# sjpark0905/DNA-LDPC-codes

Hardware: NVIDIA B200
Metric: decoded Gbit/s, n=18432 prprp (higher is better)
Workload: dtype f64

## Files before the change

dna-ldpc-codes_b200/csrc/bp_kernels.cuh:

```cuda
#pragma once
#include <cuda_runtime.h>
#include <stdint.h>

#include "bp_math.cuh"
#include "rng.cuh"

namespace dnaldpc {

constexpr int kFG = 32;

template <typename T> __device__ __forceinline__ T ld_stream(const T *p) { return __ldcs(p); }
template <typename T> __device__ __forceinline__ void st_stream(T *p, T v) { __stcs(p, v); }


template <typename T>
__device__ __noinline__ void row_slow_path(T *base, const T *lr_lane, const int32_t *cols, int deg, bool fresh) {
    auto pr_at = [&](int k) -> T { return fresh ? lr_lane[(size_t)cols[k] * kFG] : base[(size_t)k * kFG]; };
    T B = T(1);
    for (int k = deg - 1; k >= 0; k--) {
        T F = T(1);
        for (int m = 0; m < k; m++) F = mul_rn(F, check_factor_slow(pr_at(m)));
        const T dk = check_factor_slow(pr_at(k));
        base[(size_t)k * kFG] = check_to_bit_slow(mul_rn(F, B));
        B = mul_rn(B, dk);
// ... 324 lines not shown
    ck = __hiloint2double((int)w[17], (int)w[16]);
}

__device__ __forceinline__ int nth_set_bit8(uint32_t m, int r) {
    int f = 0;
#pragma unroll
    for (int q = 0; q < 8; q++) {
        if (q == r && m) f = __ffs(m) - 1;
        m &= m - 1;
    }
    return f;
}

constexpr int kTmWarps = 12;

template <int DC, int UR>
__global__ void __launch_bounds__(kTmWarps * 32, 1)
row_pass_tmem_kernel(double *__restrict__ msg, const double *__restrict__ lratio, const uint32_t *__restrict__ actw,
                     const uint32_t *__restrict__ freshw, const int32_t *__restrict__ col_idx, int M, int N, int E,
                     int g0, int G, unsigned int *__restrict__ job_counter, int l2_hint) {
    static_assert(DC % 8 == 0 && (DC / 8) * kTmBlockCols * (kTmWarps / 4) <= 512, "tensor-memory columns");
    constexpr uint32_t kTileBytes = DC * kFG * sizeof(double);
    constexpr int NB = DC / 8, NT = DC / 4, NI = (DC + 31) / 32;
    extern __shared__ __align__(128) unsigned char smem_raw[];
    const int lane = threadIdx.x & 31, warp = threadIdx.x >> 5;
    double *tile = reinterpret_cast<double *>(smem_raw) + (size_t)warp * DC * kFG;
    unsigned char *aux = smem_raw + (size_t)kTmWarps * DC * kFG * sizeof(double);
    uint64_t *bar = reinterpret_cast<uint64_t *>(aux) + warp;
    int *sidx = reinterpret_cast<int *>(aux + kTmWarps * sizeof(uint64_t)) + warp * DC;
    uint32_t *tm_slot = reinterpret_cast<uint32_t *>(aux + kTmWarps * sizeof(uint64_t) + (size_t)kTmWarps * DC * sizeof(int));
    const double *col = tile + lane;
    const uint64_t policy = l2_evict_first_policy();
    if (warp == 0) tmem_alloc_512(tm_slot);
    if (lane == 0) {
        mbar_init(bar, 1);
        mbar_fence_init();
    }
    asm volatile("tcgen05.fence::before_thread_sync;" ::: "memory");
    __syncthreads();
    asm volatile("tcgen05.fence::after_thread_sync;" ::: "memory");
    const uint32_t tm_base = *tm_slot;
    const uint32_t taddr = tm_base + ((uint32_t)((warp & 3) * 32) << 16) + (uint32_t)((warp >> 2) * NB * kTmBlockCols);
    const unsigned njobs = (unsigned)M * (unsigned)G;
    const int kq = lane >> 3, rk = lane & 7;
    uint32_t phase = 0;

    auto start_item = [&](int g, int e0, uint32_t act, uint32_t fw, double (&v)[NT]) {
        const uint32_t fresh_mask = fw & act;
        if ((act & ~fresh_mask) != 0 && lane == 0) {
            asm volatile("fence.proxy.async.shared::cta;" ::: "memory");
            mbar_expect_tx(bar, kTileBytes);
            if (l2_hint) tma_load_1d_hint(tile, msg + ((size_t)g * E + e0) * kFG, kTileBytes, bar, policy);
            else tma_load_1d(tile, msg + ((size_t)g * E + e0) * kFG, kTileBytes, bar);
        }
        if (fresh_mask != 0) {
            const bool mine = rk < __popc(fresh_mask);
            const int f = nth_set_bit8(fresh_mask, rk);
            const double *lr_base = lratio + (size_t)g * N * kFG;
#pragma unroll
            for (int t = 0; t < NT; t++) v[t] = mine ? lr_base[(size_t)sidx[t * 4 + kq] * kFG + f] : 0.0;
        }
    };
    auto claim_raw = [&]() -> unsigned {
        unsigned j = 0;
        if (lane == 0) j = atomicAdd(job_counter, 1u);
        return j;
    };

    unsigned job = __shfl_sync(0xffffffffu, claim_raw(), 0);
    unsigned job_n = __shfl_sync(0xffffffffu, claim_raw(), 0);
    int g = 0, e0 = 0;
    uint32_t act = 0, fw = 0;
    double v[NT];
    if (job < njobs) {
        g = g0 + (int)(job / (unsigned)M);
        e0 = (int)(job % (unsigned)M) * DC;
        for (int k = lane; k < DC; k += 32) sidx[k] = __ldg(col_idx + e0 + k);
        __syncwarp();
        act = actw[g]; fw = freshw[g];
        if (act != 0) start_item(g, e0, act, fw, v);
    }
    while (job < njobs) {
        const unsigned raw_nn = claim_raw();
        const bool valid_n = job_n < njobs;
        const int g_n = g0 + (int)(job_n / (unsigned)M), e0_n = (int)(job_n % (unsigned)M) * DC;
        uint32_t act_n = 0, fw_n = 0;
        int idx_n[NI];
#pragma unroll
        for (int q = 0; q < NI; q++) idx_n[q] = 0;
        if (valid_n) {
            act_n = actw[g_n]; fw_n = freshw[g_n];
#pragma unroll
            for (int q = 0; q < NI; q++)
                if (lane + 32 * q < DC) idx_n[q] = __ldg(col_idx + e0_n + lane + 32 * q);
        }
        const bool on = (act >> lane) & 1u, fresh = (fw >> lane) & 1u;
        double *base = msg + ((size_t)g * E + e0) * kFG + lane;
        const double *lr_lane = lratio + (size_t)g * N * kFG + lane;
        const int32_t *cols_cur = col_idx + e0;
        bool bad = false;
        if (act != 0) {
            const uint32_t fresh_mask = fw & act;
            if ((act & ~fresh_mask) != 0) {
                mbar_wait(bar, phase);
                phase ^= 1u;
            }
            if (fresh_mask != 0) {
                const int nf = __popc(fresh_mask);
                {
                    const bool mine = rk < nf;
                    const int f = nth_set_bit8(fresh_mask, rk);
#pragma unroll
                    for (int t = 0; t < NT; t++)
                        if (mine) tile[(t * 4 + kq) * kFG + f] = v[t];
                }
                for (int r0 = 8; r0 < nf; r0 += 8) {
                    const int r = r0 + rk;
                    const bool mine = r < nf;
                    const int f = mine ? (int)__fns(fresh_mask, 0, r + 1) : 0;
                    double w[NT];
#pragma unroll
                    for (int t = 0; t < NT; t++) w[t] = mine ? lr_lane[(size_t)sidx[t * 4 + kq] * kFG + (f - lane)] : 0.0;
#pragma unroll
                    for (int t = 0; t < NT; t++)
                        if (mine) tile[(t * 4 + kq) * kFG + f] = w[t];
                }
                __syncwarp();
            }
            double B = 1.0;
#pragma unroll(UR)
            for (int b = NB - 1; b >= 0; b--) {
                double d8[8];
                const double ckb = B;
#pragma unroll
                for (int kk = 7; kk >= 0; kk--) {
                    const double dk = check_factor(col[(b * 8 + kk) * kFG], bad);
                    d8[kk] = dk;
                    B = mul_rn(B, dk);
                }
                tmem_st_block(taddr + (uint32_t)(b * kTmBlockCols), d8, ckb);
            }
            asm volatile("tcgen05.wait::st.sync.aligned;" ::: "memory");
        }
        __syncwarp();
#pragma unroll
        for (int q = 0; q < NI; q++)
            if (lane + 32 * q < DC) sidx[lane + 32 * q] = idx_n[q];
        __syncwarp();
        if (valid_n && act_n != 0) start_item(g_n, e0_n, act_n, fw_n, v);
        if (on && bad) row_slow_path<double>(base, lr_lane, cols_cur, DC, fresh);
        if (act != 0) {
            double F = 1.0;
            const bool store = on && !bad;
#pragma unroll(UR)
            for (int b = 0; b < NB; b++) {
                double d8[8], Bv[8];
                tmem_ld_block(taddr + (uint32_t)(b * kTmBlockCols), d8, Bv[7]);
#pragma unroll
                for (int kk = 7; kk > 0; kk--) Bv[kk - 1] = mul_rn(Bv[kk], d8[kk]);
#pragma unroll
                for (int kk = 0; kk < 8; kk++) {
                    const double t = mul_rn(F, Bv[kk]);
                    const double lr = check_to_bit(t);
                    if (store) st_stream(base + (size_t)(b * 8 + kk) * kFG, lr);
                    F = mul_rn(F, d8[kk]);
                }
            }
        }
        job = job_n; g = g_n; e0 = e0_n; act = act_n; fw = fw_n;
        asm volatile("shfl.sync.idx.b32 %0, %1, 0, 31, 0xffffffff;" : "=r"(job_n) : "r"(raw_nn));
    }
    asm volatile("tcgen05.fence::before_thread_sync;" ::: "memory");
    __syncthreads();
    if (warp == 0) tmem_dealloc_512(tm_base);
}

constexpr int kColWarps = 8;

template <typename T, int DV>
struct ColIn {
    int eid[DV];
    T lr[DV];
    T P;
    int deg;
};

template <typename T, int DV, bool EXACT>
__device__ __forceinline__ void col_load(ColIn<T, DV> &c, const T *__restrict__ gmsg, const T *__restrict__ lratio,
                                         const int32_t *__restrict__ col_ptr, const int32_t *__restrict__ col_edge, int N,
                                         int g, int j, int f, bool on) {
    const int c0 = EXACT ? j * DV : __ldg(col_ptr + j);
    c.deg = EXACT ? DV : (__ldg(col_ptr + j + 1) - c0);
#pragma unroll
    for (int k = 0; k < DV; k++) c.eid[k] = (EXACT || k < c.deg) ? __ldg(col_edge + c0 + k) : 0;
#pragma unroll
    for (int k = 0; k < DV; k++) c.lr[k] = (on && (EXACT || k < c.deg)) ? ld_stream(gmsg + (size_t)c.eid[k] * kFG) : T(1);
    c.P = on ? __ldg(lratio + ((size_t)g * N + j) * kFG + f) : T(1);
}

template <typename T, int DV, bool EXACT, int ALG>
__device__ __forceinline__ bool col_finish(const ColIn<T, DV> &c, T *__restrict__ gmsg, T *__restrict__ post, int N, int g, int j,
                                           int f, bool on) {
    const int deg = c.deg;
    const int (&eid)[DV] = c.eid;
    const T (&lr)[DV] = c.lr;
    T P = c.P;
    if (ALG == ALG_MINSUM) {
        const T llr = P;
#pragma unroll
        for (int k = 0; k < DV; k++) {
            if (EXACT || k < deg) {
// ... 20 lines not shown
    if (P != P) P = T(1);
    if (post != nullptr && on) post[((size_t)g * N + j) * kFG + f] = P;
    T S = T(1);
#pragma unroll
    for (int k = DV - 1; k >= 0; k--) {
        if (EXACT || k < deg) {
            T v = mul_rn(p[k], S);
            if (v != v) v = T(1);
            if (on) st_stream(gmsg + (size_t)eid[k] * kFG, v);
            S = mul_rn(S, lr[k]);
        }
    }
    return P <= T(1);
}

template <typename T, int DV, bool EXACT, int ALG, int BITS>
__global__ void __launch_bounds__(kColWarps * 32, DV > 8 ? 1 : (BITS * DV * (int)sizeof(T) <= 64 ? 4 : (BITS * DV <= 16 ? 3 : 2)))
col_pass_kernel(T *__restrict__ msg, const T *__restrict__ lratio, uint32_t *__restrict__ decw,
                const uint32_t *__restrict__ actw, T *__restrict__ post, const int32_t *__restrict__ col_ptr,
                const int32_t *__restrict__ col_edge, int N, int E, int g0, int cols_per_warp) {
    const int lane = threadIdx.x & 31, warp = threadIdx.x >> 5;
    const int g = g0 + blockIdx.y;
    const uint32_t act = actw[g];
    if (act == 0) return;
    const bool on = (act >> lane) & 1u;
    const int jbeg = (blockIdx.x * kColWarps + warp) * cols_per_warp;
    const int jend = min(jbeg + cols_per_warp, N);
    T *gmsg = msg + (size_t)g * E * kFG + lane;
    auto put = [&](int j, bool bit) {
        const uint32_t w = __ballot_sync(0xffffffffu, bit);
        if (lane == 0) {
            uint32_t *dst = decw + (size_t)g * N + j;
            *dst = (act == 0xffffffffu) ? w : ((w & act) | (*dst & ~act));
        }
    };
    int j = jbeg;
    if (BITS > 1) {
        for (; j + BITS - 1 < jend; j += BITS) {
            ColIn<T, DV> in[BITS];
#pragma unroll
            for (int b = 0; b < BITS; b++) col_load<T, DV, EXACT>(in[b], gmsg, lratio, col_ptr, col_edge, N, g, j + b, lane, on);
#pragma unroll
            for (int b = 0; b < BITS; b++) put(j + b, col_finish<T, DV, EXACT, ALG>(in[b], gmsg, post, N, g, j + b, lane, on));
        }
    }
    for (; j < jend; j++) {
        ColIn<T, DV> a;
        col_load<T, DV, EXACT>(a, gmsg, lratio, col_ptr, col_edge, N, g, j, lane, on);
        put(j, col_finish<T, DV, EXACT, ALG>(a, gmsg, post, N, g, j, lane, on));
    }
}

struct SchedArrays {
    uint32_t *actw, *donew, *newfw, *freshw, *harvw, *unsatw;
    unsigned int *arrive;
    int32_t *slot_frame, *slot_iter, *harv_frame, *harv_iter;
    unsigned long long *next_frame;
    unsigned long long *avail;
    const int32_t *in_row, *out_row;
    unsigned long long *iter_sum;
};

__global__ void __launch_bounds__(1024)
publish_kernel(int32_t *__restrict__ in_row, int32_t *__restrict__ out_row, long long q0, int n,
               const int32_t *__restrict__ list_in, int row0_in, int row0_out, unsigned long long *avail) {
// ... 55 lines not shown
    }
}

constexpr int kSynThreads = 256;
constexpr int kSynSplit = 64;

struct SynArgs {
    int32_t *iters_out;
    uint8_t *ok_out;
    int M, N, g0, max_iter, consider_new, fixed_iters;
    unsigned int *counter;
    unsigned int *finished;
    unsigned int *counters_to_zero;
    int clear_fresh;
    unsigned int *row_jobs;
};

constexpr int kCounterWords = 4;

__device__ __forceinline__ uint32_t syn_head(const SchedArrays &s, const SynArgs &a, int g, uint32_t &act) {
    if (a.counters_to_zero && blockIdx.x == 0 && blockIdx.y == 0 && threadIdx.x == 0) {
        a.counters_to_zero[0] = 0; a.counters_to_zero[1] = 0; a.counters_to_zero[2] = 0; a.counters_to_zero[3] = 0xffffffffu;
    }
    if (a.row_jobs && blockIdx.x == 0 && blockIdx.y == 0 && threadIdx.x == 0) *a.row_jobs = 0;
    act = s.actw[g];
    const uint32_t consider = a.consider_new ? s.newfw[g] : act;
    if (consider == 0 && a.counter && blockIdx.x == 0 && threadIdx.x == 0) {
        const unsigned add = (unsigned)(__popc(act) + __popc(s.donew[g]));
        if (add) atomicAdd(a.counter, add);
    }
    return consider;
}

template <int THREADS>
__device__ __forceinline__ void syn_tail(const SchedArrays &s, const SynArgs &a, int g, uint32_t act, uint32_t consider, uint32_t acc) {
    acc = __reduce_or_sync(0xffffffffu, acc);
    __shared__ uint32_t s_or[THREADS / 32];
    __shared__ unsigned int s_ticket;
    if ((threadIdx.x & 31) == 0) s_or[threadIdx.x >> 5] = acc;
// ... 501 lines not shown
```

dna-ldpc-codes_b200/csrc/engine.cu:

```cuda
#include "engine.h"

#include <algorithm>
#include <cmath>
#include <cstdio>
#include <cstdlib>
#include <cstring>
#include <thread>

#include "../host/layers.h"
#include "bp_kernels.cuh"
#include "layered_kernels.cuh"
#include "sw_kernels.cuh"

namespace dnaldpc {

#define CK(call)                                      \
    do {                                              \
        cudaError_t e_ = (call);                      \
        if (e_ != cudaSuccess) return fail(e_, #call); \
    } while (0)

int Engine::fail(cudaError_t e, const char *what) {
    err_ = std::string("CUDA error: ") + cudaGetErrorString(e) + " in " + what;
    return DNALDPC_ERR_CUDA;
// ... 75 lines not shown
    if (own_stream_) cudaStreamDestroy(own_stream_);
    for (auto &s : io_stream_) if (s) cudaStreamDestroy(s);
}

int Engine::ensure_slots(int G, bool want_post) {
    if (G > cap_groups_) {
        void *ptrs[] = {d_msg_, d_lratio_, d_post_, d_decw_, d_masks_, d_arrive_, d_slot_, d_mv_};
        for (void *p : ptrs) if (p) cudaFree(p);
        d_msg_ = d_lratio_ = d_post_ = nullptr; d_decw_ = d_masks_ = nullptr; d_arrive_ = nullptr; d_slot_ = d_mv_ = nullptr;
        cap_groups_ = 0;
        const size_t msg_elems = std::max<size_t>((size_t)E_, (size_t)M_ * layer_w_);
        CK(cudaMalloc(&d_msg_, std::max<size_t>((size_t)G * msg_elems * kFG * esz_, 16)));
        CK(cudaMalloc(&d_lratio_, (size_t)G * N_ * kFG * esz_));
        CK(cudaMalloc((void **)&d_decw_, (size_t)G * N_ * sizeof(uint32_t)));
        CK(cudaMalloc((void **)&d_masks_, (size_t)G * 6 * sizeof(uint32_t)));
        CK(cudaMalloc((void **)&d_arrive_, (size_t)G * sizeof(unsigned)));
        CK(cudaMalloc((void **)&d_slot_, (size_t)G * kFG * 4 * sizeof(int32_t)));
        CK(cudaMalloc((void **)&d_mv_, ((size_t)G * kFG * 2 + 2) * sizeof(int32_t)));
        cap_groups_ = G;
    }
    if (want_post && !d_post_) CK(cudaMalloc(&d_post_, (size_t)cap_groups_ * N_ * kFG * esz_));
    return DNALDPC_OK;
}

int Engine::ensure_frame_scratch(int64_t F) {
    if (F > cap_frames_) {
        if (d_iters_) cudaFree(d_iters_);
        if (d_ok_) cudaFree(d_ok_);
        d_iters_ = nullptr; d_ok_ = nullptr; cap_frames_ = 0;
        CK(cudaMalloc((void **)&d_iters_, (size_t)F * sizeof(int32_t)));
        CK(cudaMalloc((void **)&d_ok_, (size_t)F));
// ... 5 lines not shown
void Engine::fill_sched(SchedArrays &s) const {
    const size_t G = (size_t)cap_groups_;
    s.actw = d_masks_; s.donew = d_masks_ + G; s.newfw = d_masks_ + 2 * G; s.freshw = d_masks_ + 3 * G;
    s.harvw = d_masks_ + 4 * G; s.unsatw = d_masks_ + 5 * G;
    s.arrive = d_arrive_;
    const size_t S = G * kFG;
    s.slot_frame = d_slot_; s.slot_iter = d_slot_ + S; s.harv_frame = d_slot_ + 2 * S; s.harv_iter = d_slot_ + 3 * S;
    s.next_frame = d_next_;
    s.avail = d_next_ + 1;
    s.iter_sum = d_next_ + 2;
    s.in_row = d_rows_;
    s.out_row = d_rows_ + cap_rows_;
}


template <typename T> int Engine::launch_row(int g0, int G, cudaStream_t st) {
    T *msg = (T *)d_msg_;
    const T *lr = (const T *)d_lratio_;
    SchedArrays s;
    fill_sched(s);
    const long long items = (long long)G * M_;
    const unsigned grid = (unsigned)((items + kRowWarps - 1) / kRowWarps);
#define ROW(DC, EX)                                                                                                                       \
    do {                                                                                                                                  \
        if (minsum_) row_pass_kernel<T, DC, EX, ALG_MINSUM><<<grid, kRowWarps * 32, 0, st>>>(msg, lr, s.actw, s.freshw, d_row_ptr_, d_col_idx_, M_, N_, E_, g0, G); \
        else row_pass_kernel<T, DC, EX, ALG_BP><<<grid, kRowWarps * 32, 0, st>>>(msg, lr, s.actw, s.freshw, d_row_ptr_, d_col_idx_, M_, N_, E_, g0, G);         \
    } while (0)
    static const bool no_smem = getenv("DNALDPC_ROW_REGS") != nullptr;
    static const bool steady_only = getenv("DNALDPC_ROW_SMEM_STEADY_ONLY") != nullptr;
    const bool use_smem = !no_smem && (steady_ || !steady_only) && !minsum_ && sizeof(T) == 8;
    static const bool use_tmem = getenv("DNALDPC_ROW_NO_TMEM") == nullptr;
    static const int tm_hint = getenv("DNALDPC_ROW_L2HINT") ? atoi(getenv("DNALDPC_ROW_L2HINT")) : 1;
    if (use_smem && use_tmem && reg_rows_ && max_row_deg_ == 72) {
        const size_t smem = (size_t)kTmWarps * 72 * kFG * sizeof(double) + kTmWarps * sizeof(uint64_t) + (size_t)kTmWarps * 72 * sizeof(int) + 16;
        static const int ur_env = getenv("DNALDPC_ROW_UNROLL") ? atoi(getenv("DNALDPC_ROW_UNROLL")) : 0;
        const int ur = ur_env ? ur_env : (steady_ ? 9 : 3);
        if (!tmem_attr_set_) {
            CK(cudaFuncSetAttribute(row_pass_tmem_kernel<72, 1>, cudaFuncAttributeMaxDynamicSharedMemorySize, (int)smem));
            CK(cudaFuncSetAttribute(row_pass_tmem_kernel<72, 3>, cudaFuncAttributeMaxDynamicSharedMemorySize, (int)smem));
            CK(cudaFuncSetAttribute(row_pass_tmem_kernel<72, 9>, cudaFuncAttributeMaxDynamicSharedMemorySize, (int)smem));
            tmem_attr_set_ = true;
        }
        const unsigned pgrid = (unsigned)std::min<long long>((long long)sm_count_, (items + kTmWarps - 1) / kTmWarps);
        unsigned *jobs = d_counters_ + (size_t)kRing * kCounterWords;
#define TMROW(U) row_pass_tmem_kernel<72, U><<<pgrid, kTmWarps * 32, smem, st>>>((double *)msg, (const double *)lr, s.actw, s.freshw, d_col_idx_, M_, N_, E_, g0, G, jobs, tm_hint)
        if (ur == 9) TMROW(9);
        else if (ur == 3) TMROW(3);
        else TMROW(1);
#undef TMROW
    } else if (use_smem && reg_rows_ && max_row_deg_ == 72) {
        const size_t smem = (size_t)kRowWarps * 72 * kFG * sizeof(T) + kRowWarps * sizeof(uint64_t);
        bool &attr_set = smem_attr_set_[sizeof(T) == 4];
        if (!attr_set) {
            CK(cudaFuncSetAttribute(row_pass_smem_kernel<T, 72>, cudaFuncAttributeMaxDynamicSharedMemorySize, (int)smem));
            attr_set = true;
        }
        row_pass_smem_kernel<T, 72><<<grid, kRowWarps * 32, smem, st>>>(msg, lr, s.actw, s.freshw, d_row_ptr_, d_col_idx_, M_, N_, E_, g0, G);
    } else if (use_smem && max_row_deg_ <= 32 && max_row_deg_ > 8) {
        const size_t smem = (size_t)kRowWarps * 32 * kFG * sizeof(T) + kRowWarps * sizeof(uint64_t);
// ... 62 lines not shown
        stats.kernel_launches++;
    }
    CK(cudaGetLastError());
    return DNALDPC_OK;
}

int Engine::launch_syndrome(const dnaldpc_output &out, int G, int max_iter, int consider_new, int fixed, unsigned *counter,
                            unsigned *finished, unsigned *rearm, int clear_fresh, cudaStream_t st) {
    SchedArrays s;
    fill_sched(s);
    SynArgs a;
    a.iters_out = out.iters; a.ok_out = out.is_codeword;
    a.M = M_; a.N = N_; a.g0 = 0; a.max_iter = max_iter; a.consider_new = consider_new; a.fixed_iters = fixed;
    a.counter = counter; a.finished = finished; a.counters_to_zero = rearm; a.clear_fresh = clear_fresh;
    a.row_jobs = d_counters_ + (size_t)kRing * kCounterWords;
    const size_t smem = (size_t)N_ * sizeof(uint32_t);
    static const bool no_smem = getenv("DNALDPC_SYN_GATHER") != nullptr;
    if (!no_smem && smem <= (size_t)kSynSmemGate && N_ % 4 == 0) {
        if (!syn_attr_set_) {
            CK(cudaFuncSetAttribute(syndrome_update_smem_kernel, cudaFuncAttributeMaxDynamicSharedMemorySize, kSynSmemGate));
            syn_attr_set_ = true;
        }
        static const int split = getenv("DNALDPC_SYN_SPLIT") ? std::max(1, atoi(getenv("DNALDPC_SYN_SPLIT"))) : kSynSmemSplit;
        syndrome_update_smem_kernel<<<dim3((unsigned)split, (unsigned)G), kSynSmemThreads, smem, st>>>(d_decw_, s, a, d_row_ptr_, d_col_idx_);
    } else if (!no_smem && (size_t)N_ * sizeof(uint16_t) <= (size_t)kSynHalfGate && N_ % 4 == 0) {
        if (!syn_half_attr_set_) {
            CK(cudaFuncSetAttribute(syndrome_update_half_kernel, cudaFuncAttributeMaxDynamicSharedMemorySize, kSynHalfGate));
            syn_half_attr_set_ = true;
        }
        syndrome_update_half_kernel<<<dim3(kSynSmemSplit, (unsigned)G, 2), kSynSmemThreads, (size_t)N_ * sizeof(uint16_t), st>>>(d_decw_, s, a, d_row_ptr_, d_col_idx_);
// ... 166 lines not shown
                if (rc) return rc;
                rc = launch_syndrome(out, G, ss.max_iter, round == 2, fixed, round == 2 ? cnt : nullptr, cnt + 2,
                                     round == 1 ? rearm : nullptr, 0, st);
                if (rc) return rc;
            }
        } else {
            rc = launch_syndrome(out, G, ss.max_iter, 0, fixed, cnt, cnt + 2, rearm, 1, st);
            if (rc) return rc;
        }
        CK(cudaMemcpyAsync(h_counters_ + kCounterWords * (tick % kRing), cnt, kCounterWords * sizeof(unsigned), cudaMemcpyDeviceToHost, st));
        CK(cudaEventRecord(ev_[tick % kRing], st));
        if (tick >= kLag) {
            const long long t = tick - kLag;
            CK(cudaEventSynchronize(ev_[t % kRing]));
            const unsigned *hc = h_counters_ + kCounterWords * (t % kRing);
            last_inuse = hc[0]; last_admitted = hc[1]; last_finished = hc[2];
            admitted_total += last_admitted;
            if (admit_ring[t % kRing]) low_water = std::min<long long>(hc[3] == 0xffffffffu ? admitted_total : (long long)hc[3], admitted_total);
            if (final && admitted_total == published() && last_inuse == 0) break;
            steady_ = last_admitted == 0 && last_inuse >= (unsigned)S;
            if (!final && last_inuse == 0 && admitted_total == published()) {
                src.wait_for_frames();
                last_admitted = 1;
            }
            if (!no_compact && !profiling && !(layered_ && empty_cols_) && final && admitted_total == published() && packed_cap >= 2 * kFG &&
                (long long)last_inuse * 100 <= packed_cap * compact_pct) {
                int32_t *mv_src = d_mv_, *mv_dst = d_mv_ + (size_t)cap_groups_ * kFG, *mv_cnt = d_mv_ + (size_t)cap_groups_ * kFG * 2;
                compact_plan_kernel<<<1, 32, 0, st>>>(s, G, mv_src, mv_dst, mv_cnt);
                const int msg_elems = layered_ ? M_ * layer_w_ : E_;
                dim3 mgrid((unsigned)((msg_elems + N_ + kMoveThreads * kMoveUnroll - 1) / (kMoveThreads * kMoveUnroll)),
                           (unsigned)std::min<unsigned>(std::max(last_inuse, 1u), 2048u));
                compact_move_kernel<T><<<mgrid, kMoveThreads, 0, st>>>((T *)d_msg_, (T *)d_lratio_, mv_src, mv_dst, mv_cnt, N_, msg_elems);
                stats.kernel_launches += 2;
                stats.compactions++;
                CK(cudaGetLastError());
                G_rc = (int)std::min<long long>(G, ((long long)last_inuse + kFG - 1) / kFG);
                G_rc = std::max(G_rc, 1);
                packed_cap = (long long)G_rc * kFG;
            }
        }
        const bool trace = trace_ticks_ > 0 && tick >= 8 && tick < 8 + kTrace && tick < 8 + trace_ticks_;
        if (trace) CK(cudaEventRecord(trace_ev_[3 * (tick - 8)], st));
        if (profiling) CK(cudaEventRecord(prof_ev_[0], st));
        rc = layered_ ? launch_layers<T>(G_rc, st) : launch_row<T>(0, G_rc, st);
        if (rc) return rc;
        if (profiling) CK(cudaEventRecord(prof_ev_[1], st));
        if (trace) CK(cudaEventRecord(trace_ev_[3 * (tick - 8) + 1], st));
        if (!layered_) rc = launch_col<T>(0, G_rc, want_post, st);
        if (rc) return rc;
        if (trace) { CK(cudaEventRecord(trace_ev_[3 * (tick - 8) + 2], st)); traced_ = (int)(tick - 8) + 1; }
        if (profiling) {
            CK(cudaEventRecord(prof_ev_[2], st));
            CK(cudaEventSynchronize(prof_ev_[2]));
            float a_ms = 0, b_ms = 0;
            cudaEventElapsedTime(&a_ms, prof_ev_[0], prof_ev_[1]);
            cudaEventElapsedTime(&b_ms, prof_ev_[1], prof_ev_[2]);
            stats.row_ms += a_ms;
            stats.col_ms += b_ms;
            stats.waves++;
        }
    }
    unsigned long long it_sum = 0;
    CK(cudaMemcpyAsync(&it_sum, d_next_ + 2, sizeof(it_sum), cudaMemcpyDeviceToHost, st));
// ... 498 lines not shown
```

dna-ldpc-codes_b200/csrc/engine.h:

```cpp
#pragma once
#include <cuda_runtime.h>

#include <atomic>
#include <cstdint>
#include <string>
#include <vector>

#include "../../include/dnaldpc.h"
#include "../host/code.h"

namespace dnaldpc {

struct SchedArrays;
class Engine;

struct Session {
    dnaldpc_input in;
    dnaldpc_output out;
    int max_iter = 0;
    int64_t max_frames = 0;
};

class FrameSource {
  public:
// ... 28 lines not shown
                   double read_err, int8_t *out_k, cudaStream_t stream, uint64_t cw_off = 0);

    dnaldpc_stats stats{};
    bool profiling = false;
    double minsum_scale = 1.0;
    int trace_ticks_ = 0;
    int trace_result(double *row_ms, double *col_ms, double *sched_ms);

  private:
    template <typename T> int run(const Session &ss, FrameSource &src, cudaStream_t st);
    int sw_groups(const Code &code, const dnaldpc_window &w, const std::vector<int> &sched, const double *lratio, int64_t F,
                  int max_iter, const dnaldpc_output &out, int G);
    int sw_lockstep(const dnaldpc_window &w, const std::vector<int> &sched, const double *lratio, int64_t F, int max_iter,
                    const dnaldpc_output &out, int G);
    int ensure_rows(int64_t frames);
    template <typename T> int launch_row(int g0, int G, cudaStream_t st);
    template <typename T> int launch_col(int g0, int G, bool want_post, cudaStream_t st);
    template <typename T> int launch_layers(int G, cudaStream_t st);
    template <typename T> int launch_harvest_setup(const dnaldpc_input &in, const dnaldpc_output &out, int g0, int G, cudaStream_t st);
    int launch_syndrome(const dnaldpc_output &out, int G, int max_iter, int consider_new, int fixed, unsigned *counter,
                        unsigned *finished, unsigned *rearm, int clear_fresh, cudaStream_t st);
    int ensure_slots(int groups, bool want_post);
    int ensure_frame_scratch(int64_t F);
    int fail(cudaError_t e, const char *what);
    int fail(const std::string &m, int rc);
    void fill_sched(SchedArrays &s) const;

    std::string err_;
    int device_ = 0, precision_ = 0, wave_frames_ = 4096, sm_count_ = 148;
    int M_ = 0, N_ = 0, E_ = 0, max_row_deg_ = 0, max_col_deg_ = 0;
    bool reg_rows_ = false, reg_cols_ = false;
    bool smem_attr_set_[2] = {false, false}, syn_attr_set_ = false, tmem_attr_set_ = false, syn_half_attr_set_ = false;
    bool steady_ = false;
    bool minsum_ = false;
    bool layered_ = false;
    size_t esz_ = 8;
    int32_t *d_row_ptr_ = nullptr, *d_col_idx_ = nullptr, *d_col_ptr_ = nullptr, *d_col_edge_ = nullptr;
    int32_t *d_layer_rows_ = nullptr;
    std::vector<int32_t> layer_ptr_;
    int layer_w_ = 0;
    bool empty_cols_ = false;
    int cap_groups_ = 0;
    void *d_msg_ = nullptr, *d_lratio_ = nullptr, *d_post_ = nullptr;
    uint32_t *d_decw_ = nullptr, *d_masks_ = nullptr;
    unsigned int *d_arrive_ = nullptr;
    int32_t *d_slot_ = nullptr;
    void *d_sw_lr_ = nullptr;
// ... 60 lines not shown
```

Before: 0.2377.

## Fuse check-node and bit-node passes into one persistent kernel with per-group counters

Adds a fused kernel that interleaves check-row items and bit-column items through a single atomic job queue. Bit items of group g wait on a per-group completion counter, using acquire/release and a timeout, until every check row of that group is done. A lead window and proportional interleaving order the work so one group's bit work overlaps the next group's check work. This removes the separate column launch and the idle tail between the two passes. Check messages are stored with an L2 evict_last hint and read back with relaxed coherent loads, which adds spin-wait, timeout and deadlock risk.

```diff
diff --git a/dna-ldpc-codes_b200/csrc/bp_kernels.cuh b/dna-ldpc-codes_b200/csrc/bp_kernels.cuh
--- a/dna-ldpc-codes_b200/csrc/bp_kernels.cuh
+++ b/dna-ldpc-codes_b200/csrc/bp_kernels.cuh
@@ -3,6 +3,7 @@
 #include <stdint.h>
 
 #include "bp_math.cuh"
+#include "fused_order.h"
 #include "rng.cuh"
 
 namespace dnaldpc {
@@ -362,11 +363,63 @@
 
 constexpr int kTmWarps = 12;
 
-template <int DC, int UR>
-__global__ void __launch_bounds__(kTmWarps * 32, 1)
-row_pass_tmem_kernel(double *__restrict__ msg, const double *__restrict__ lratio, const uint32_t *__restrict__ actw,
-                     const uint32_t *__restrict__ freshw, const int32_t *__restrict__ col_idx, int M, int N, int E,
-                     int g0, int G, unsigned int *__restrict__ job_counter, int l2_hint) {
+template <typename T, int DV, bool EXACT, int ALG, int BITS, bool COH = false>
+__device__ __forceinline__ void col_warp(T *__restrict__ msg, const T *__restrict__ lratio, uint32_t *__restrict__ decw,
+                                         uint32_t act, T *__restrict__ post, const int32_t *__restrict__ col_ptr,
+                                         const int32_t *__restrict__ col_edge, int N, int E, int g, int jbeg, int jend, int lane);
+
+struct FuseArgs {
+    uint32_t *decw;
+    double *post;
+    const int32_t *col_edge;
+    unsigned int *done;
+    unsigned int *err;
+    int NB, lead;
+    int keep;
+};
+constexpr int kFuseBits = 2;
+constexpr int kFuseLead = 2048;
+constexpr unsigned long long kFuseWaitNs = 2000000000ull;
+
+__device__ __forceinline__ uint64_t l2_evict_last_policy() {
+    uint64_t p;
+    asm volatile("createpolicy.fractional.L2::evict_last.b64 %0, 1.0;" : "=l"(p));
+    return p;
+}
+__device__ __forceinline__ void st_hint(double *p, double v, uint64_t policy) {
+    asm volatile("st.global.L2::cache_hint.f64 [%0], %1, %2;" ::"l"(p), "d"(v), "l"(policy) : "memory");
+}
+__device__ __forceinline__ unsigned ld_acquire_gpu(const unsigned *p) {
+    unsigned v;
+    asm volatile("ld.acquire.gpu.global.u32 %0, [%1];" : "=r"(v) : "l"(p) : "memory");
+    return v;
+}
+__device__ __forceinline__ void red_release_gpu_add(unsigned *p, unsigned v) {
+    asm volatile("red.release.gpu.global.add.u32 [%0], %1;" ::"l"(p), "r"(v) : "memory");
+}
+__device__ __forceinline__ unsigned long long global_ns() {
+    unsigned long long t;
+    asm volatile("mov.u64 %0, %%globaltimer;" : "=l"(t));
+    return t;
+}
+__device__ __noinline__ bool wait_count(const unsigned *ctr, unsigned target, unsigned *err) {
+    if (ld_acquire_gpu(ctr) >= target) return true;
+    const unsigned long long t0 = global_ns();
+    for (;;) {
+        __nanosleep(128);
+        if (ld_acquire_gpu(ctr) >= target) return true;
+        if (*(volatile unsigned *)err != 0u) return false;
+        if (global_ns() - t0 > kFuseWaitNs) {
+            atomicOr(err, 1u);
+            return false;
+        }
+    }
+}
+
+template <int DC, int UR, bool FUSED>
+__device__ __forceinline__ void tmem_pass(double *__restrict__ msg, const double *__restrict__ lratio, const uint32_t *__restrict__ actw,
+                                          const uint32_t *__restrict__ freshw, const int32_t *__restrict__ col_idx, int M, int N, int E,
+                                          int g0, int G, unsigned int *__restrict__ job_counter, int l2_hint, const FuseArgs &fa) {
     static_assert(DC % 8 == 0 && (DC / 8) * kTmBlockCols * (kTmWarps / 4) <= 512, "tensor-memory columns");
     constexpr uint32_t kTileBytes = DC * kFG * sizeof(double);
     constexpr int NB = DC / 8, NT = DC / 4, NI = (DC + 31) / 32;
@@ -379,6 +432,7 @@
     uint32_t *tm_slot = reinterpret_cast<uint32_t *>(aux + kTmWarps * sizeof(uint64_t) + (size_t)kTmWarps * DC * sizeof(int));
     const double *col = tile + lane;
     const uint64_t policy = l2_evict_first_policy();
+    const uint64_t keep = FUSED ? (fa.keep ? l2_evict_last_policy() : policy) : 0;
     if (warp == 0) tmem_alloc_512(tm_slot);
     if (lane == 0) {
         mbar_init(bar, 1);
@@ -389,10 +443,22 @@
     asm volatile("tcgen05.fence::after_thread_sync;" ::: "memory");
     const uint32_t tm_base = *tm_slot;
     const uint32_t taddr = tm_base + ((uint32_t)((warp & 3) * 32) << 16) + (uint32_t)((warp >> 2) * NB * kTmBlockCols);
-    const unsigned njobs = (unsigned)M * (unsigned)G;
+    const unsigned njobs = FUSED ? fused_items(G, M, fa.NB) : (unsigned)M * (unsigned)G;
     const int kq = lane >> 3, rk = lane & 7;
     uint32_t phase = 0;
 
+    auto decode = [&](unsigned j, bool &bit, int &g, int &e0) {
+        if (FUSED) {
+            const FusedItem it = fused_item(j, G, M, fa.NB, fa.lead);
+            bit = it.bit != 0;
+            g = g0 + it.g;
+            e0 = bit ? it.idx : it.idx * DC;
+        } else {
+            bit = false;
+            g = g0 + (int)(j / (unsigned)M);
+            e0 = (int)(j % (unsigned)M) * DC;
+        }
+    };
     auto start_item = [&](int g, int e0, uint32_t act, uint32_t fw, double (&v)[NT]) {
         const uint32_t fresh_mask = fw & act;
         if ((act & ~fresh_mask) != 0 && lane == 0) {
@@ -418,109 +484,155 @@
     unsigned job = __shfl_sync(0xffffffffu, claim_raw(), 0);
     unsigned job_n = __shfl_sync(0xffffffffu, claim_raw(), 0);
     int g = 0, e0 = 0;
+    bool bit = false;
     uint32_t act = 0, fw = 0;
     double v[NT];
     if (job < njobs) {
-        g = g0 + (int)(job / (unsigned)M);
-        e0 = (int)(job % (unsigned)M) * DC;
-        for (int k = lane; k < DC; k += 32) sidx[k] = __ldg(col_idx + e0 + k);
-        __syncwarp();
+        decode(job, bit, g, e0);
+        if (!bit) {
+            for (int k = lane; k < DC; k += 32) sidx[k] = __ldg(col_idx + e0 + k);
+            __syncwarp();
+        }
         act = actw[g]; fw = freshw[g];
-        if (act != 0) start_item(g, e0, act, fw, v);
+        if (!bit && act != 0) start_item(g, e0, act, fw, v);
     }
     while (job < njobs) {
         const unsigned raw_nn = claim_raw();
         const bool valid_n = job_n < njobs;
-        const int g_n = g0 + (int)(job_n / (unsigned)M), e0_n = (int)(job_n % (unsigned)M) * DC;
+        bool bit_n;
+        int g_n, e0_n;
+        decode(job_n, bit_n, g_n, e0_n);
         uint32_t act_n = 0, fw_n = 0;
         int idx_n[NI];
 #pragma unroll
         for (int q = 0; q < NI; q++) idx_n[q] = 0;
         if (valid_n) {
             act_n = actw[g_n]; fw_n = freshw[g_n];
+            if (!bit_n) {
+#pragma unroll
+                for (int q = 0; q < NI; q++)
+                    if (lane + 32 * q < DC) idx_n[q] = __ldg(col_idx + e0_n + lane + 32 * q);
+            }
+        }
+        auto start_next = [&]() {
 #pragma unroll
             for (int q = 0; q < NI; q++)
-                if (lane + 32 * q < DC) idx_n[q] = __ldg(col_idx + e0_n + lane + 32 * q);
-        }
-        const bool on = (act >> lane) & 1u, fresh = (fw >> lane) & 1u;
-        double *base = msg + ((size_t)g * E + e0) * kFG + lane;
-        const double *lr_lane = lratio + (size_t)g * N * kFG + lane;
-        const int32_t *cols_cur = col_idx + e0;
-        bool bad = false;
-        if (act != 0) {
-            const uint32_t fresh_mask = fw & act;
-            if ((act & ~fresh_mask) != 0) {
-                mbar_wait(bar, phase);
-                phase ^= 1u;
-            }
-            if (fresh_mask != 0) {
-                const int nf = __popc(fresh_mask);
-                {
-                    const bool mine = rk < nf;
-                    const int f = nth_set_bit8(fresh_mask, rk);
-#pragma unroll
-                    for (int t = 0; t < NT; t++)
-                        if (mine) tile[(t * 4 + kq) * kFG + f] = v[t];
+                if (lane + 32 * q < DC) sidx[lane + 32 * q] = idx_n[q];
+            __syncwarp();
+            if (valid_n && !bit_n && act_n != 0) start_item(g_n, e0_n, act_n, fw_n, v);
+        };
+        if (FUSED && bit) {
+            start_next();
+            if (act != 0) {
+                bool ok = true;
+                if (lane == 0) ok = wait_count(fa.done + g, (unsigned)M, fa.err);
+                __syncwarp();
+                if (__shfl_sync(0xffffffffu, (int)ok, 0)) {
+                    const int jbeg = e0 * 8;
+                    col_warp<double, 8, true, ALG_BP, kFuseBits, true>(msg, lratio, fa.decw, act, fa.post, nullptr, fa.col_edge, N, E,
+                                                                      g, jbeg, min(jbeg + 8, N), lane);
                 }
-                for (int r0 = 8; r0 < nf; r0 += 8) {
-                    const int r = r0 + rk;
-                    const bool mine = r < nf;
-                    const int f = mine ? (int)__fns(fresh_mask, 0, r + 1) : 0;
-                    double w[NT];
-#pragma unroll
-                    for (int t = 0; t < NT; t++) w[t] = mine ? lr_lane[(size_t)sidx[t * 4 + kq] * kFG + (f - lane)] : 0.0;
-#pragma unroll
-                    for (int t = 0; t < NT; t++)
-                        if (mine) tile[(t * 4 + kq) * kFG + f] = w[t];
+            }
+        } else {
+            const bool on = (act >> lane) & 1u, fresh = (fw >> lane) & 1u;
+            double *base = msg + ((size_t)g * E + e0) * kFG + lane;
+            const double *lr_lane = lratio + (size_t)g * N * kFG + lane;
+            const int32_t *cols_cur = col_idx + e0;
+            bool bad = false;
+            if (act != 0) {
+                const uint32_t fresh_mask = fw & act;
+                if ((act & ~fresh_mask) != 0) {
+                    mbar_wait(bar, phase);
+                    phase ^= 1u;
                 }
+                if (fresh_mask != 0) {
+                    const int nf = __popc(fresh_mask);
+                    {
+                        const bool mine = rk < nf;
+                        const int f = nth_set_bit8(fresh_mask, rk);
+#pragma unroll
+                        for (int t = 0; t < NT; t++)
+                            if (mine) tile[(t * 4 + kq) * kFG + f] = v[t];
+                    }
+                    for (int r0 = 8; r0 < nf; r0 += 8) {
+                        const int r = r0 + rk;
+                        const bool mine = r < nf;
+                        const int f = mine ? (int)__fns(fresh_mask, 0, r + 1) : 0;
+                        double w[NT];
+#pragma unroll
+                        for (int t = 0; t < NT; t++) w[t] = mine ? lr_lane[(size_t)sidx[t * 4 + kq] * kFG + (f - lane)] : 0.0;
+#pragma unroll
+                        for (int t = 0; t < NT; t++)
+                            if (mine) tile[(t * 4 + kq) * kFG + f] = w[t];
+                    }
+                    __syncwarp();
+                }
+                double B = 1.0;
+#pragma unroll(UR)
+                for (int b = NB - 1; b >= 0; b--) {
+                    double d8[8];
+                    const double ckb = B;
+#pragma unroll
+                    for (int kk = 7; kk >= 0; kk--) {
+                        const double dk = check_factor(col[(b * 8 + kk) * kFG], bad);
+                        d8[kk] = dk;
+                        B = mul_rn(B, dk);
+                    }
+                    tmem_st_block(taddr + (uint32_t)(b * kTmBlockCols), d8, ckb);
+                }
+                asm volatile("tcgen05.wait::st.sync.aligned;" ::: "memory");
+            }
+            __syncwarp();
+            start_next();
+            if (on && bad) row_slow_path<double>(base, lr_lane, cols_cur, DC, fresh);
+            if (act != 0) {
+                double F = 1.0;
+                const bool store = on && !bad;
+#pragma unroll(UR)
+                for (int b = 0; b < NB; b++) {
+                    double d8[8], Bv[8];
+                    tmem_ld_block(taddr + (uint32_t)(b * kTmBlockCols), d8, Bv[7]);
+#pragma unroll
+                    for (int kk = 7; kk > 0; kk--) Bv[kk - 1] = mul_rn(Bv[kk], d8[kk]);
+#pragma unroll
+                    for (int kk = 0; kk < 8; kk++) {
+                        const double t = mul_rn(F, Bv[kk]);
+                        const double lr = check_to_bit(t);
+                        if (store) {
+                            if (FUSED) st_hint(base + (size_t)(b * 8 + kk) * kFG, lr, keep);
+                            else st_stream(base + (size_t)(b * 8 + kk) * kFG, lr);
+                        }
+                        F = mul_rn(F, d8[kk]);
+                    }
+                }
+            }
+            if (FUSED) {
                 __syncwarp();
-            }
-            double B = 1.0;
-#pragma unroll(UR)
-            for (int b = NB - 1; b >= 0; b--) {
-                double d8[8];
-                const double ckb = B;
-#pragma unroll
-                for (int kk = 7; kk >= 0; kk--) {
-                    const double dk = check_factor(col[(b * 8 + kk) * kFG], bad);
-                    d8[kk] = dk;
-                    B = mul_rn(B, dk);
-                }
-                tmem_st_block(taddr + (uint32_t)(b * kTmBlockCols), d8, ckb);
-            }
-            asm volatile("tcgen05.wait::st.sync.aligned;" ::: "memory");
-        }
-        __syncwarp();
-#pragma unroll
-        for (int q = 0; q < NI; q++)
-            if (lane + 32 * q < DC) sidx[lane + 32 * q] = idx_n[q];
-        __syncwarp();
-        if (valid_n && act_n != 0) start_item(g_n, e0_n, act_n, fw_n, v);
-        if (on && bad) row_slow_path<double>(base, lr_lane, cols_cur, DC, fresh);
-        if (act != 0) {
-            double F = 1.0;
-            const bool store = on && !bad;
-#pragma unroll(UR)
-            for (int b = 0; b < NB; b++) {
-                double d8[8], Bv[8];
-                tmem_ld_block(taddr + (uint32_t)(b * kTmBlockCols), d8, Bv[7]);
-#pragma unroll
-                for (int kk = 7; kk > 0; kk--) Bv[kk - 1] = mul_rn(Bv[kk], d8[kk]);
-#pragma unroll
-                for (int kk = 0; kk < 8; kk++) {
-                    const double t = mul_rn(F, Bv[kk]);
-                    const double lr = check_to_bit(t);
-                    if (store) st_stream(base + (size_t)(b * 8 + kk) * kFG, lr);
-                    F = mul_rn(F, d8[kk]);
-                }
-            }
-        }
-        job = job_n; g = g_n; e0 = e0_n; act = act_n; fw = fw_n;
+                if (lane == 0) red_release_gpu_add(fa.done + g, 1u);
+            }
+        }
+        job = job_n; g = g_n; e0 = e0_n; act = act_n; fw = fw_n; bit = bit_n;
         asm volatile("shfl.sync.idx.b32 %0, %1, 0, 31, 0xffffffff;" : "=r"(job_n) : "r"(raw_nn));
     }
     asm volatile("tcgen05.fence::before_thread_sync;" ::: "memory");
     __syncthreads();
     if (warp == 0) tmem_dealloc_512(tm_base);
+}
+
+template <int DC, int UR>
+__global__ void __launch_bounds__(kTmWarps * 32, 1)
+row_pass_tmem_kernel(double *__restrict__ msg, const double *__restrict__ lratio, const uint32_t *__restrict__ actw,
+                     const uint32_t *__restrict__ freshw, const int32_t *__restrict__ col_idx, int M, int N, int E,
+                     int g0, int G, unsigned int *__restrict__ job_counter, int l2_hint) {
+    tmem_pass<DC, UR, false>(msg, lratio, actw, freshw, col_idx, M, N, E, g0, G, job_counter, l2_hint, FuseArgs{});
+}
+
+template <int UR>
+__global__ void __launch_bounds__(kTmWarps * 32, 1)
+tick_fused_kernel(double *__restrict__ msg, const double *__restrict__ lratio, const uint32_t *__restrict__ actw,
+                  const uint32_t *__restrict__ freshw, const int32_t *__restrict__ col_idx, int M, int N, int E,
+                  int g0, int G, unsigned int *__restrict__ job_counter, int l2_hint, FuseArgs fa) {
+    tmem_pass<72, UR, true>(msg, lratio, actw, freshw, col_idx, M, N, E, g0, G, job_counter, l2_hint, fa);
 }
 
 constexpr int kColWarps = 8;
@@ -533,7 +645,19 @@
     int deg;
 };
 
-template <typename T, int DV, bool EXACT>
+template <typename T> __device__ __forceinline__ T ld_coherent(const T *p);
+template <> __device__ __forceinline__ double ld_coherent<double>(const double *p) {
+    double v;
+    asm volatile("ld.relaxed.gpu.global.f64 %0, [%1];" : "=d"(v) : "l"(p));
+    return v;
+}
+template <> __device__ __forceinline__ float ld_coherent<float>(const float *p) {
+    float v;
+    asm volatile("ld.relaxed.gpu.global.f32 %0, [%1];" : "=f"(v) : "l"(p));
+    return v;
+}
+
+template <typename T, int DV, bool EXACT, bool COH = false>
 __device__ __forceinline__ void col_load(ColIn<T, DV> &c, const T *__restrict__ gmsg, const T *__restrict__ lratio,
                                          const int32_t *__restrict__ col_ptr, const int32_t *__restrict__ col_edge, int N,
                                          int g, int j, int f, bool on) {
@@ -542,7 +666,8 @@
 #pragma unroll
     for (int k = 0; k < DV; k++) c.eid[k] = (EXACT || k < c.deg) ? __ldg(col_edge + c0 + k) : 0;
 #pragma unroll
-    for (int k = 0; k < DV; k++) c.lr[k] = (on && (EXACT || k < c.deg)) ? ld_stream(gmsg + (size_t)c.eid[k] * kFG) : T(1);
+    for (int k = 0; k < DV; k++)
+        c.lr[k] = (on && (EXACT || k < c.deg)) ? (COH ? ld_coherent(gmsg + (size_t)c.eid[k] * kFG) : ld_stream(gmsg + (size_t)c.eid[k] * kFG)) : T(1);
     c.P = on ? __ldg(lratio + ((size_t)g * N + j) * kFG + f) : T(1);
 }
 
@@ -593,6 +718,36 @@
     return P <= T(1);
 }
 
+template <typename T, int DV, bool EXACT, int ALG, int BITS, bool COH>
+__device__ __forceinline__ void col_warp(T *__restrict__ msg, const T *__restrict__ lratio, uint32_t *__restrict__ decw,
+                                         uint32_t act, T *__restrict__ post, const int32_t *__restrict__ col_ptr,
+                                         const int32_t *__restrict__ col_edge, int N, int E, int g, int jbeg, int jend, int lane) {
+    const bool on = (act >> lane) & 1u;
+    T *gmsg = msg + (size_t)g * E * kFG + lane;
+    auto put = [&](int j, bool bit) {
+        const uint32_t w = __ballot_sync(0xffffffffu, bit);
+        if (lane == 0) {
+            uint32_t *dst = decw + (size_t)g * N + j;
+            *dst = (act == 0xffffffffu) ? w : ((w & act) | (*dst & ~act));
+        }
+    };
+    int j = jbeg;
+    if (BITS > 1) {
+        for (; j + BITS - 1 < jend; j += BITS) {
+            ColIn<T, DV> in[BITS];
+#pragma unroll
+            for (int b = 0; b < BITS; b++) col_load<T, DV, EXACT, COH>(in[b], gmsg, lratio, col_ptr, col_edge, N, g, j + b, lane, on);
+#pragma unroll
+            for (int b = 0; b < BITS; b++) put(j + b, col_finish<T, DV, EXACT, ALG>(in[b], gmsg, post, N, g, j + b, lane, on));
+        }
+    }
+    for (; j < jend; j++) {
+        ColIn<T, DV> a;
+        col_load<T, DV, EXACT, COH>(a, gmsg, lratio, col_ptr, col_edge, N, g, j, lane, on);
+        put(j, col_finish<T, DV, EXACT, ALG>(a, gmsg, post, N, g, j, lane, on));
+    }
+}
+
 template <typename T, int DV, bool EXACT, int ALG, int BITS>
 __global__ void __launch_bounds__(kColWarps * 32, DV > 8 ? 1 : (BITS * DV * (int)sizeof(T) <= 64 ? 4 : (BITS * DV <= 16 ? 3 : 2)))
 col_pass_kernel(T *__restrict__ msg, const T *__restrict__ lratio, uint32_t *__restrict__ decw,
@@ -602,32 +757,9 @@
     const int g = g0 + blockIdx.y;
     const uint32_t act = actw[g];
     if (act == 0) return;
-    const bool on = (act >> lane) & 1u;
     const int jbeg = (blockIdx.x * kColWarps + warp) * cols_per_warp;
     const int jend = min(jbeg + cols_per_warp, N);
-    T *gmsg = msg + (size_t)g * E * kFG + lane;
-    auto put = [&](int j, bool bit) {
-        const uint32_t w = __ballot_sync(0xffffffffu, bit);
-        if (lane == 0) {
-            uint32_t *dst = decw + (size_t)g * N + j;
-            *dst = (act == 0xffffffffu) ? w : ((w & act) | (*dst & ~act));
-        }
-    };
-    int j = jbeg;
-    if (BITS > 1) {
-        for (; j + BITS - 1 < jend; j += BITS) {
-            ColIn<T, DV> in[BITS];
-#pragma unroll
-            for (int b = 0; b < BITS; b++) col_load<T, DV, EXACT>(in[b], gmsg, lratio, col_ptr, col_edge, N, g, j + b, lane, on);
-#pragma unroll
-            for (int b = 0; b < BITS; b++) put(j + b, col_finish<T, DV, EXACT, ALG>(in[b], gmsg, post, N, g, j + b, lane, on));
-        }
-    }
-    for (; j < jend; j++) {
-        ColIn<T, DV> a;
-        col_load<T, DV, EXACT>(a, gmsg, lratio, col_ptr, col_edge, N, g, j, lane, on);
-        put(j, col_finish<T, DV, EXACT, ALG>(a, gmsg, post, N, g, j, lane, on));
-    }
+    col_warp<T, DV, EXACT, ALG, BITS>(msg, lratio, decw, act, post, col_ptr, col_edge, N, E, g, jbeg, jend, lane);
 }
 
 struct SchedArrays {
@@ -713,15 +845,18 @@
     unsigned int *counters_to_zero;
     int clear_fresh;
     unsigned int *row_jobs;
+    unsigned int *chk_done;
 };
 
-constexpr int kCounterWords = 4;
+constexpr int kCounterWords = 5;
 
 __device__ __forceinline__ uint32_t syn_head(const SchedArrays &s, const SynArgs &a, int g, uint32_t &act) {
     if (a.counters_to_zero && blockIdx.x == 0 && blockIdx.y == 0 && threadIdx.x == 0) {
         a.counters_to_zero[0] = 0; a.counters_to_zero[1] = 0; a.counters_to_zero[2] = 0; a.counters_to_zero[3] = 0xffffffffu;
+        a.counters_to_zero[4] = 0;
     }
     if (a.row_jobs && blockIdx.x == 0 && blockIdx.y == 0 && threadIdx.x == 0) *a.row_jobs = 0;
+    if (a.chk_done && blockIdx.x == 0 && threadIdx.x == 0) a.chk_done[g] = 0;
     act = s.actw[g];
     const uint32_t consider = a.consider_new ? s.newfw[g] : act;
     if (consider == 0 && a.counter && blockIdx.x == 0 && threadIdx.x == 0) {
diff --git a/dna-ldpc-codes_b200/csrc/engine.cu b/dna-ldpc-codes_b200/csrc/engine.cu
--- a/dna-ldpc-codes_b200/csrc/engine.cu
+++ b/dna-ldpc-codes_b200/csrc/engine.cu
@@ -113,7 +113,7 @@
         CK(cudaMalloc(&d_lratio_, (size_t)G * N_ * kFG * esz_));
         CK(cudaMalloc((void **)&d_decw_, (size_t)G * N_ * sizeof(uint32_t)));
         CK(cudaMalloc((void **)&d_masks_, (size_t)G * 6 * sizeof(uint32_t)));
-        CK(cudaMalloc((void **)&d_arrive_, (size_t)G * sizeof(unsigned)));
+        CK(cudaMalloc((void **)&d_arrive_, (size_t)G * 2 * sizeof(unsigned)));
         CK(cudaMalloc((void **)&d_slot_, (size_t)G * kFG * 4 * sizeof(int32_t)));
         CK(cudaMalloc((void **)&d_mv_, ((size_t)G * kFG * 2 + 2) * sizeof(int32_t)));
         cap_groups_ = G;
@@ -149,7 +149,8 @@
 }
 
 
-template <typename T> int Engine::launch_row(int g0, int G, cudaStream_t st) {
+template <typename T> int Engine::launch_row(int g0, int G, bool want_post, unsigned *err_word, bool *fused, cudaStream_t st) {
+    *fused = false;
     T *msg = (T *)d_msg_;
     const T *lr = (const T *)d_lratio_;
     SchedArrays s;
@@ -176,8 +177,32 @@
             CK(cudaFuncSetAttribute(row_pass_tmem_kernel<72, 9>, cudaFuncAttributeMaxDynamicSharedMemorySize, (int)smem));
             tmem_attr_set_ = true;
         }
+        unsigned *jobs = d_counters_ + (size_t)kRing * kCounterWords;
+        static const bool no_fuse = getenv("DNALDPC_NO_FUSE") != nullptr && atoi(getenv("DNALDPC_NO_FUSE")) != 0;
+        static const int lead = getenv("DNALDPC_FUSE_LEAD") ? std::max(0, atoi(getenv("DNALDPC_FUSE_LEAD"))) : kFuseLead;
+        static const int keep = getenv("DNALDPC_FUSE_L2KEEP") ? atoi(getenv("DNALDPC_FUSE_L2KEEP")) : 1;
+        const int nb = (N_ + 7) / 8;
+        if (!no_fuse && reg_cols_ && max_col_deg_ == 8 && (long long)(M_ + nb) * M_ < (1LL << 31)) {
+            if (!fused_attr_set_) {
+                CK(cudaFuncSetAttribute(tick_fused_kernel<3>, cudaFuncAttributeMaxDynamicSharedMemorySize, (int)smem));
+                CK(cudaFuncSetAttribute(tick_fused_kernel<9>, cudaFuncAttributeMaxDynamicSharedMemorySize, (int)smem));
+                fused_attr_set_ = true;
+            }
+            FuseArgs fa;
+            fa.decw = d_decw_; fa.post = want_post ? (double *)d_post_ : nullptr; fa.col_edge = d_col_edge_;
+            fa.done = d_arrive_ + cap_groups_; fa.err = err_word; fa.NB = nb; fa.lead = lead; fa.keep = keep;
+            const long long fitems = (long long)G * (M_ + nb);
+            const unsigned fgrid = (unsigned)std::min<long long>((long long)sm_count_, (fitems + kTmWarps - 1) / kTmWarps);
+#define TMFUSE(U) tick_fused_kernel<U><<<fgrid, kTmWarps * 32, smem, st>>>((double *)msg, (const double *)lr, s.actw, s.freshw, d_col_idx_, M_, N_, E_, g0, G, jobs, tm_hint, fa)
+            if (ur == 9) TMFUSE(9);
+            else TMFUSE(3);
+#undef TMFUSE
+            *fused = true;
+            stats.kernel_launches++;
+            CK(cudaGetLastError());
+            return DNALDPC_OK;
+        }
         const unsigned pgrid = (unsigned)std::min<long long>((long long)sm_count_, (items + kTmWarps - 1) / kTmWarps);
-        unsigned *jobs = d_counters_ + (size_t)kRing * kCounterWords;
 #define TMROW(U) row_pass_tmem_kernel<72, U><<<pgrid, kTmWarps * 32, smem, st>>>((double *)msg, (const double *)lr, s.actw, s.freshw, d_col_idx_, M_, N_, E_, g0, G, jobs, tm_hint)
         if (ur == 9) TMROW(9);
         else if (ur == 3) TMROW(3);
@@ -270,6 +295,7 @@
     a.M = M_; a.N = N_; a.g0 = 0; a.max_iter = max_iter; a.consider_new = consider_new; a.fixed_iters = fixed;
     a.counter = counter; a.finished = finished; a.counters_to_zero = rearm; a.clear_fresh = clear_fresh;
     a.row_jobs = d_counters_ + (size_t)kRing * kCounterWords;
+    a.chk_done = d_arrive_ + cap_groups_;
     const size_t smem = (size_t)N_ * sizeof(uint32_t);
     static const bool no_smem = getenv("DNALDPC_SYN_GATHER") != nullptr;
     if (!no_smem && smem <= (size_t)kSynSmemGate && N_ % 4 == 0) {
@@ -466,6 +492,7 @@
             const long long t = tick - kLag;
             CK(cudaEventSynchronize(ev_[t % kRing]));
             const unsigned *hc = h_counters_ + kCounterWords * (t % kRing);
+            if (hc[4]) return fail("fused check/bit pass: a bit item waited more than 2 s for its group's check items (set DNALDPC_NO_FUSE=1 to run the two-launch path)", DNALDPC_ERR_CUDA);
             last_inuse = hc[0]; last_admitted = hc[1]; last_finished = hc[2];
             admitted_total += last_admitted;
             if (admit_ring[t % kRing]) low_water = std::min<long long>(hc[3] == 0xffffffffu ? admitted_total : (long long)hc[3], admitted_total);
@@ -494,11 +521,12 @@
         const bool trace = trace_ticks_ > 0 && tick >= 8 && tick < 8 + kTrace && tick < 8 + trace_ticks_;
         if (trace) CK(cudaEventRecord(trace_ev_[3 * (tick - 8)], st));
         if (profiling) CK(cudaEventRecord(prof_ev_[0], st));
-        rc = layered_ ? launch_layers<T>(G_rc, st) : launch_row<T>(0, G_rc, st);
+        bool fused = false;
+        rc = layered_ ? launch_layers<T>(G_rc, st) : launch_row<T>(0, G_rc, want_post, cnt + 4, &fused, st);
         if (rc) return rc;
         if (profiling) CK(cudaEventRecord(prof_ev_[1], st));
         if (trace) CK(cudaEventRecord(trace_ev_[3 * (tick - 8) + 1], st));
-        if (!layered_) rc = launch_col<T>(0, G_rc, want_post, st);
+        if (!layered_ && !fused) rc = launch_col<T>(0, G_rc, want_post, st);
         if (rc) return rc;
         if (trace) { CK(cudaEventRecord(trace_ev_[3 * (tick - 8) + 2], st)); traced_ = (int)(tick - 8) + 1; }
         if (profiling) {
diff --git a/dna-ldpc-codes_b200/csrc/engine.h b/dna-ldpc-codes_b200/csrc/engine.h
--- a/dna-ldpc-codes_b200/csrc/engine.h
+++ b/dna-ldpc-codes_b200/csrc/engine.h
@@ -66,7 +66,7 @@
     int sw_lockstep(const dnaldpc_window &w, const std::vector<int> &sched, const double *lratio, int64_t F, int max_iter,
                     const dnaldpc_output &out, int G);
     int ensure_rows(int64_t frames);
-    template <typename T> int launch_row(int g0, int G, cudaStream_t st);
+    template <typename T> int launch_row(int g0, int G, bool want_post, unsigned *err_word, bool *fused, cudaStream_t st);
     template <typename T> int launch_col(int g0, int G, bool want_post, cudaStream_t st);
     template <typename T> int launch_layers(int G, cudaStream_t st);
     template <typename T> int launch_harvest_setup(const dnaldpc_input &in, const dnaldpc_output &out, int g0, int G, cudaStream_t st);
@@ -83,6 +83,7 @@
     int M_ = 0, N_ = 0, E_ = 0, max_row_deg_ = 0, max_col_deg_ = 0;
     bool reg_rows_ = false, reg_cols_ = false;
     bool smem_attr_set_[2] = {false, false}, syn_attr_set_ = false, tmem_attr_set_ = false, syn_half_attr_set_ = false;
+    bool fused_attr_set_ = false;
     bool steady_ = false;
     bool minsum_ = false;
     bool layered_ = false;
diff --git a/dna-ldpc-codes_b200/csrc/fused_order.h b/dna-ldpc-codes_b200/csrc/fused_order.h
--- /dev/null
+++ b/dna-ldpc-codes_b200/csrc/fused_order.h
@@ -0,0 +1,36 @@
+#pragma once
+
+#if defined(__CUDACC__)
+#define DNALDPC_HD __host__ __device__ __forceinline__
+#else
+#define DNALDPC_HD inline
+#endif
+
+namespace dnaldpc {
+
+struct FusedItem {
+    int bit;
+    int g;
+    int idx;
+};
+
+DNALDPC_HD unsigned fused_items(int G, int M, int NB) { return (unsigned)G * (unsigned)(M + NB); }
+
+DNALDPC_HD FusedItem fused_item(unsigned t, int G, int M, int NB, int lead) {
+    FusedItem it;
+    if (t < (unsigned)M) { it.bit = 0; it.g = 0; it.idx = (int)t; return it; }
+    t -= (unsigned)M;
+    const unsigned seg_len = (unsigned)(M + NB);
+    const int s = 1 + (int)(t / seg_len);
+    const unsigned r = t % seg_len;
+    if (s == G) { it.bit = 1; it.g = G - 1; it.idx = (int)r; return it; }
+    const unsigned w = lead < M ? (unsigned)lead : (unsigned)M;
+    if (r < w) { it.bit = 0; it.g = s; it.idx = (int)r; return it; }
+    const unsigned q = r - w, R = (unsigned)M - w, L = R + (unsigned)NB;
+    const unsigned nc = q * R / L, nc1 = (q + 1) * R / L;
+    if (nc1 > nc) { it.bit = 0; it.g = s; it.idx = (int)(w + nc); }
+    else { it.bit = 1; it.g = s - 1; it.idx = (int)(q - nc); }
+    return it;
+}
+
+}
```

Result: slower. 0.2032 (median of 6 runs) (-14.5%).
